# blasif/cocons

Measured on AMD Instinct MI355X. Metric: -2loglik evals/sec (dense cov_rns + Cholesky/solve/log-det, fp64) at n=10000, higher is better.
Workload: dtype f64

## Files before the change

### cocons_amd/csrc/api.hip

```cpp
#include "fit.hpp"

thread_local std::string g_err;

int fail(int code, const char *fmt, ...)
{
    char buf[512];
    va_list ap;
    va_start(ap, fmt);
    vsnprintf(buf, sizeof buf, fmt, ap);
    va_end(ap);
    g_err = buf;
    return code;
}

extern "C" const char *cocons_last_error(void) { return g_err.c_str(); }
extern "C" int cocons_abi_version(void) { return 1; }

extern "C" int cocons_device_count(void)
{
    int n = 0;
    hipError_t e = hipGetDeviceCount(&n);
    if (e != hipSuccess) { g_err = hipGetErrorString(e); return -1; }
    return n;
}
// ... 271 lines not shown
        CK(hipMemcpyAsync(f->dxb, x_betas, (size_t)n * q * sizeof(double), hipMemcpyHostToDevice, f->stream));
    }
    CK(hipStreamSynchronize(f->stream));
    CK(f->dloc.alloc((size_t)LOCP_FIELDS * f->npad));
    CK(f->dinv.alloc(2 * 8 * 256));
    int nr_max = r + (q > p ? q : p);
    f->out_cap = (size_t)(1 + nr_max * nr_max) * (size_t)(f->nt + 2);
    {
        double *hbase = nullptr;
        CK(f->dinfo_out.alloc(f->out_cap + 1));
        CK(hipHostMalloc(&hbase, (f->out_cap + 2) * sizeof(double)));
        f->dinfo = (int *)f->dinfo_out.get(); f->dout = f->dinfo_out + 1;
        f->hinfo = (int *)hbase; f->hout = hbase + 1;
        f->hinfo_init = (int *)(hbase + 1 + f->out_cap);
        f->hinfo_init[0] = 0x7f7f7f7f; f->hinfo_init[1] = 0;
    }
    for (auto &e : f->ev) CK(hipEventCreate(&e));
    f->engine_ok = want_engine;
    CK(hipEventCreateWithFlags(&f->ev_eng, hipEventDisableTiming));
    if (!defer_matrix && fit_alloc_matrix(f, nr_max) != 0) { cocons_fit_destroy(f); return nullptr; }
#undef CK
    if (engine_warm(f) != 0) { cocons_fit_destroy(f); return nullptr; }
    if (return_locked) f->op_mu.lock();
    registry_add(f);
    return f;
}

extern "C" cocons_fit *cocons_fit_create(int n, int p, int r, int q, const double *locs,
                                         const double *X, const double *z, const double *x_betas,
                                         const double *smooth_limits, int device)
// ... 215 lines not shown
    FIT_ENTER(f);
    HIPCHK(hipStreamSynchronize(f->stream));
    if (f->stream2) HIPCHK(hipStreamSynchronize(f->stream2));
    if (f->own_stream) { HIPCHK(hipStreamDestroy(f->stream)); f->own_stream = false; }
    f->stream = (hipStream_t)stream;
    return 0;
}

extern "C" int cocons_fit_sync(cocons_fit *f)
{
    FIT_ENTER(f);
    HIPCHK(hipStreamSynchronize(f->stream));
    return 0;
}

void assemble_sigma(cocons_fit *f, const double *theta, int which, int col0, int col1)
{
    ThetaVecs tv;
    make_theta_vecs(theta, f->p, tv);
    ModeSel ms = select_mode(theta, f->p, f->smooth_limits, which);
    launch_loc_params(loc_args(f->n, f->p, f->dX, f->dlocs, f->dloc, f->npad, tv, ms.smooth_kind, f->smooth_limits), f->stream);
    PairArgs pa;
    memset(&pa, 0, sizeof pa);
    pa.n = f->n; pa.m = f->n;
    pa.rows = f->dloc; pa.cols = f->dloc;
    pa.stride = f->npad; pa.stride_rows = f->npad;
    pa.out = f->dA; pa.ld = f->lda;
    pa.nrows_out = f->npad; pa.ncols_out = col1;
    pa.bj0 = col0 / 64;
    if (pa.bj0 < f->pad0 / 64) pa.bj0 = f->pad0 / 64;
    pa.pad_diag = f->nslot > 0 ? 1e300 : 1.0;
    pa.gr = ms.gr; pa.nu_fixed = ms.nu_fixed;
    launch_pair_sym(ms.mode, false, pa, f->stream);
}

int assemble_sigma_taper(cocons_fit *f, const double *theta)
{
    ThetaVecs tv;
    make_theta_vecs(theta, f->p, tv, true);
    ModeSel ms = select_mode(theta, f->p, f->smooth_limits, 0);
    launch_loc_params(loc_args(f->n, f->p, f->dX, f->dlocs, f->dloc, f->npad, tv, ms.smooth_kind, f->smooth_limits), f->stream);
    if (f->d_thi) launch_band_zero(f->dA, f->lda, f->d_thi, f->nt, f->taper_maxband, f->stream, f->skew);
    else HIPCHK(hipMemsetAsync(f->dA, 0, f->lda * (size_t)f->npad * sizeof(double), f->stream));
    TaperLaunch t;
    t.mode = ms.mode; t.nrows = f->n; t.nnz = f->taper_nnz; t.ci = f->d_tci; t.rp = f->d_trp; t.nu_fixed = ms.nu_fixed;
    t.rows = t.cols = f->dloc; t.stride_rows = t.stride = f->npad;
    t.tapv = f->d_tval; t.A = f->dA; t.lda = f->lda; t.skew = f->skew; t.npad = f->npad;
    launch_taper(t, f->stream);
    launch_pad_identity(f->dA, f->lda, f->n, f->npad, f->stream, f->skew);
    return 0;
}

int no_taper(cocons_fit *f, const char *who)
{
    if (f->taper_nnz > 0) return fail(-1, "%s: not available on a taper fit (cocons_neg2loglik_dense is)", who);
    return 0;
}

void assemble_rhs(cocons_fit *f, const double *mean, bool use_trend, const double *xb, int nxb,
                  int col0, int col1, bool zero_rest, bool slots)
{
    if (slots) { zero_rest = false; col1 = f->n; }
    RhsArgs ra;
    memset(&ra, 0, sizeof ra);
    ra.n = f->n; ra.p = f->p; ra.X = f->dX; ra.ldx = f->n;
    ra.use_trend = use_trend ? 1 : 0;
    if (use_trend) for (int i = 0; i < f->p; ++i) ra.mean[i] = canon_nan(mean[i]);
    ra.src = f->dz; ra.lds = f->n;
    ra.out = f->dA; ra.ld = f->lda;
    ra.skew = f->skew; ra.npad = f->npad;
    ra.row0 = slots ? f->n : f->npad; ra.nrows = f->r;
    ra.nrows_zero = (nxb > 0 || !zero_rest) ? 0 : f->rhs_act - f->r;
    ra.col0 = col0; ra.ncols_out = col1;
    launch_rhs_rows(ra, f->stream);
    if (nxb > 0) {
        ra.use_trend = 0;
        ra.src = xb; ra.lds = f->n;
        ra.row0 = (slots ? f->n : f->npad) + f->r; ra.nrows = nxb;
        ra.nrows_zero = zero_rest ? f->rhs_act - f->r - nxb : 0;
        launch_rhs_rows(ra, f->stream);
    }
}

FactorView main_view(cocons_fit *f)
{
    FactorView v;
    v.A = f->dA; v.lda = f->lda; v.nt = f->nt; v.mt = f->nt + f->rhs_act / TILE;
    v.hi = f->taper_hi.empty() ? nullptr : f->taper_hi.data();
    v.skew = f->skew;
    return v;
}

static RhsLayout rhs_layout(const cocons_fit *f, int nrhs)
{
    RhsLayout l;
    l.slots = f->nslot >= nrhs && f->nslot > 0;
// ... 149 lines not shown

static void count_update_flops(cocons_fit *f, int kw, int t0)
{
    double m = (double)f->n_user - ((double)t0 * TILE - (double)f->pad0);
    if (m > (double)f->n_user) m = (double)f->n_user;
    if (m < 0) m = 0;
    const double K = (double)kw * TILE - (t0 == kw ? (double)f->pad0 : 0.0);
    f->upd_flops += K * m * (m + 1.0) + 2.0 * K * (double)f->nrhs_cur * m;
}

static bool engine_wanted(cocons_fit *f, const FactorView &v)
{
    return engine_enabled() && f->engine_ok && f->stream2 != nullptr && f->engine_skip == 0 && v.nt > 4;
}

int flags_reset(cocons_fit *f, int nt)
{
    if (f->flags_cap < nt) {
        const int cap = round_up(nt + 8, 64);
        HIPCHK(f->dflags.reserve(handoff_word_count(cap), f->stream, f->stream2));
        f->flags_cap = cap;
    }
    HIPCHK(hipMemsetAsync(f->dflags, 0, handoff_word_count(f->flags_cap) * sizeof(unsigned), f->stream));
    return 0;
}

int mbox_reset(cocons_fit *f, int nt, bool engine_schedule)
{
    const MboxLayout l = mbox_layout(nt, tun().panel_fused && tun().engine_pair, tun().panel_split != 0);
    HIPCHK(f->dmbox.reserve(l.total(), f->stream, f->stream2));
    f->mbox = l;
    HIPCHK(hipMemsetAsync(f->dmbox, 0xff, (engine_schedule ? l.total() : l.tiles) * sizeof(double), f->stream));
    return 0;
}

static int engine_warm(cocons_fit *f)
{
    if (!engine_enabled() || f->nt <= 4 || !f->engine_ok) { f->engine_ok = f->engine_ok && f->stream2 != nullptr; return 0; }
    if (!f->stream2) HIPCHK(hipStreamCreateWithFlags(&f->stream2, hipStreamNonBlocking));
    if (int rc = flags_reset(f, f->nt)) return rc;
    HIPCHK(hipStreamSynchronize(f->stream));
    {
        std::vector<hipStream_t> losers;
        int ok = 0;
        for (int attempt = 0; attempt < 8; ++attempt) {
            ok = streams_run_concurrently(f->stream2, f->stream, handoff_words(f).selftest);
            if (ok != 0) break;
            losers.push_back(f->stream2);
            f->stream2 = nullptr;
// ... 87 lines not shown
                                                tun().dag_order ? tun().dag_bw : 0, tun().dag_bh);
        HIPCHK(hipStreamSynchronize(f->stream));
        if (f->stream2) HIPCHK(hipStreamSynchronize(f->stream2));
        HIPCHK(f->ddag_steps.reserve(steps.size() + 1, f->stream, f->stream2, -1, true));
        HIPCHK(hipMemcpyAsync(f->ddag_steps, steps.data(), steps.size() * sizeof(DagStepHost), hipMemcpyHostToDevice, f->stream));
        HIPCHK(f->ddag_ftab.reserve(ftab.size(), f->stream, f->stream2));
        if (!ftab.empty())
            HIPCHK(hipMemcpyAsync(f->ddag_ftab, ftab.data(), ftab.size() * sizeof(unsigned), hipMemcpyHostToDevice, f->stream));
        f->dag_xcd_g = want_tab ? xcd_g : 0;
        f->dag_have_ftab = want_tab && !ftab.empty();
        HIPCHK(hipStreamSynchronize(f->stream));
        f->dag_nsteps = (int)steps.size(); f->dag_ntasks = ntasks;
        memcpy(f->dag_key, key, sizeof key);
        HIPCHK(f->ddag.reserve(dag_words(f, v.mt).total, f->stream, f->stream2));
    }
    HIPCHK(hipMemsetAsync(f->ddag, 0, f->ddag.count() * sizeof(unsigned), f->stream));
    const size_t trace_elems = dag_trace_words(f, v.nt).count;
    if (tun().dag_trace) HIPCHK(f->ddag_trace.reserve(trace_elems, f->stream, f->stream2));
    f->dag_trace_tasks = (tun().dag_trace && f->ddag_trace) ? f->dag_ntasks : 0;
    if (f->dag_trace_tasks)
        HIPCHK(hipMemsetAsync(f->ddag_trace, 0, trace_elems * sizeof(unsigned long long), f->stream));
    return 0;
}

extern "C" long long cocons_debug_dag_trace(cocons_fit *f, int *nsteps_out, int *steps_out, unsigned long long *stamps_out,
                                            unsigned long long *engine_out)
{
    FIT_ENTER(f);
    if (!f->ddag_steps) return fail(-1, "cocons_debug_dag_trace: no DAG factorisation on this handle yet");
    if (nsteps_out) *nsteps_out = f->dag_nsteps;
    HIPCHK(hipStreamSynchronize(f->stream));
// ... 26 lines not shown
    const DagWords w = dag_words(f, v.mt);
    DagLaunch d;
    d.A = v.A; d.lda = v.lda; d.P = f->dP; d.Wt = f->dWt; d.steps = f->ddag_steps; d.nsteps = f->dag_nsteps; d.ntasks = f->dag_ntasks;
    d.queue = w.queue; d.tdone = w.tdone; d.pdone = w.pdone; d.pstride = w.pstride; d.pall = w.pall; d.dcount = w.dcount; d.xcnt = w.xcnt;
    d.partbuf = f->dpart; d.sig = hw.in; d.out = hw.out; d.xr = hw.xr; d.abort_word = hw.abort;
    d.alive = alive; d.xcc_quota = dag_xcc_quota(); d.xcd_g = f->dag_xcd_g;
    if (f->dag_have_ftab) d.ftab = f->ddag_ftab;
    return d;
}

static int engine_start(cocons_fit *f, const FactorView &v)
{
    if (f->engine_live) return 0;
    const int nt = v.nt;
    hipStream_t M = f->stream;
    if (int rc = flags_reset(f, nt)) return rc;
    f->dag_next = dag_wanted(f, v);
    if (f->dag_next) {
        if (int rc = dag_prepare(f, v)) return rc;
        if (f->dag_nsteps < 2) f->dag_next = false;
    }
    f->engine_pair_live = tun().engine_pair != 0 ? 1 : 0;
    if (f->engine_pair_live || (tun().potrf_follow && !f->follow_off))
        if (int rc = mbox_reset(f, nt > f->nt ? nt : f->nt)) return rc;
    HIPCHK(hipEventRecord(f->ev_eng, M));
    HIPCHK(hipStreamWaitEvent(f->stream2, f->ev_eng, 0));
    const HandoffWords hw = handoff_words(f);
    EngineLaunch e;
    e.A = v.A; e.lda = v.lda; e.nt = nt; e.dinv = f->dinv; e.info = f->dinfo; e.in_wait_ms = tun().engine_in_wait_ms;
    e.in = hw.in; e.out = hw.out; e.xr = hw.xr; e.abort_word = hw.abort; e.alive = hw.alive;
    if (f->dag_next) { e.wbuf = f->dWt; e.pbuf = f->dP; e.dag_until = 2 * f->dag_nsteps; }
    if (f->dag_next && f->dag_trace_tasks) e.trace = dag_trace_words(f, nt).engine;
    if (f->engine_pair_live) e.mbox = f->dmbox;
    launch_potrf_engine(e, f->stream2);
    f->engine_live = true;
    return 0;
}

int factorize(cocons_fit *f, const FactorView &v, std::vector<hipEvent_t> *ev_upd)
{
    const int nt = v.nt, mt = v.mt;
    hipStream_t M = f->stream;
    launch_front_identity(v.A, v.lda, f->pad0, mt * TILE, M);
    f->follow_used = false;
    if (!engine_wanted(f, v)) {
        f->engine_used = false;
        f->dag_used = false;
        if (int rc = flags_reset(f, nt)) return rc;
        if (tun().potrf_follow && !f->follow_off)
            if (int rc = mbox_reset(f, nt > f->nt ? nt : f->nt, false)) return rc;
        if (v.hi) {
            for (int k = 0; k < nt; ++k) {
                const int hb = v.hi[k] < nt ? v.hi[k] : nt;
                double *q = f->dinv + (size_t)(k & 1) * 2048;
                double *Ak = band_base(v.A, k, v.skew);
                const int e0 = v.skew ? k + v.skew : nt, e1 = e0 + (mt - nt);
                RowRange rows;
                rows.r0 = (k + 1) * TILE; rows.r1 = e1 * TILE - 64 * v.trim; rows.band_r1 = hb * TILE; rows.ext_r0 = e0 * TILE;
                potrf_solve(f, Ak, v.lda, k, rows, q, M);
                if (k + 1 < nt) {
                    UpdateLaunch u = v.update(hb);
                    u.panel_in_c(k * TILE); u.K = TILE; u.ti0 = k + 1; u.ti1 = mt; u.tj0 = k + 1; u.tj1 = hb < nt ? hb : nt; u.lower_only = true;
                    u.skew = v.skew;
                    launch_update(u, M);
                }
// ... 82 lines not shown
{
    HIPCHK(hipMemcpyAsync(f->dinfo, f->hinfo_init, 2 * sizeof(int), hipMemcpyHostToDevice, f->stream));
    return 0;
}

static int enqueue_eval_impl(cocons_fit *f, const double *theta, const double *mean, bool use_trend,
                             const double *xb, int nxb, std::vector<hipEvent_t> *ev_upd, bool stage_events)
{
    const int nrhs = f->r + nxb;
    f->nrhs_cur = nrhs;
    const int was_clean = f->border_clean;
    const double *was_A = f->dA;
    if (int rc = fit_alloc_matrix(f, nrhs)) return rc;
    const bool zero_rest = !(was_clean == nrhs && was_A == f->dA);
    f->border_pending = nrhs;
    if (stage_events) hipEventRecord(f->ev[0], f->stream);
    if (int rc = reset_info(f)) return rc;
    if (f->taper_nnz > 0) { if (int rc = assemble_sigma_taper(f, theta)) return rc; }
    else assemble_sigma(f, theta, 0, 0, f->npad);
    const RhsLayout lay = rhs_layout(f, nrhs);
    const bool slots = lay.slots;
    FactorView fv = rhs_view(f, lay);
    fv.dag_ok = true;
    if (engine_wanted(f, fv))
        if (int rc = engine_start(f, fv)) return rc;
    assemble_rhs(f, mean, use_trend, xb, nxb, 0, f->npad, zero_rest, slots);
    if (stage_events) hipEventRecord(f->ev[1], f->stream);
    if (int rc = factorize(f, fv, ev_upd)) return rc;
    if (stage_events) hipEventRecord(f->ev[2], f->stream);
    launch_finalize(f->dA, f->lda, f->n, slots ? f->n : f->npad, nrhs, f->dout, f->stream, f->skew, f->npad,
                    f->dag_used ? f->dP : nullptr, f->dag_used ? 2 * TILE * f->dag_nsteps : 0);
    HIPCHK(hipMemcpyAsync(f->hinfo, f->dinfo, (size_t)(2 + nrhs * nrhs) * sizeof(double),
                          hipMemcpyDeviceToHost, f->stream));
    if (stage_events) hipEventRecord(f->ev[3], f->stream);
    HIPCHK(hipGetLastError());
    return 0;
}

static int enqueue_eval(cocons_fit *f, const double *theta, const double *mean, bool use_trend,
                        const double *xb, int nxb, std::vector<hipEvent_t> *ev_upd, bool stage_events)
{
    struct timespec t0, t1;
    clock_gettime(CLOCK_MONOTONIC, &t0);
    const int rc = enqueue_eval_impl(f, theta, mean, use_trend, xb, nxb, ev_upd, stage_events);
    clock_gettime(CLOCK_MONOTONIC, &t1);
    f->enq_host_us += (t1.tv_sec - t0.tv_sec) * 1e6 + (t1.tv_nsec - t0.tv_nsec) * 1e-3;
    f->enq_calls++;
    return rc;
// ... 726 lines not shown
```

### cocons_amd/csrc/api_shard.hip

```cpp
#include <dlfcn.h>
#include <thread>
#include "fit.hpp"

struct RcclApi {
    void *h;
    ncclResult_t (*GetUniqueId)(ncclUniqueId *);
    ncclResult_t (*CommInitRank)(ncclComm_t *, int, ncclUniqueId, int);
    ncclResult_t (*CommInitAll)(ncclComm_t *, int, const int *);
    ncclResult_t (*CommDestroy)(ncclComm_t);
    ncclResult_t (*Broadcast)(const void *, void *, size_t, ncclDataType_t, int, ncclComm_t, hipStream_t);
    ncclResult_t (*AllReduce)(const void *, void *, size_t, ncclDataType_t, ncclRedOp_t, ncclComm_t, hipStream_t);
    ncclResult_t (*AllGather)(const void *, void *, size_t, ncclDataType_t, ncclComm_t, hipStream_t);
    ncclResult_t (*GroupStart)();
    ncclResult_t (*GroupEnd)();
    const char *(*GetErrorString)(ncclResult_t);
    ncclResult_t (*CommCount)(const ncclComm_t, int *);
    ncclResult_t (*CommUserRank)(const ncclComm_t, int *);
    ncclResult_t (*CommCuDevice)(const ncclComm_t, int *);
    ncclResult_t (*CommAbort)(ncclComm_t);
    ncclResult_t (*Send)(const void *, size_t, ncclDataType_t, int, ncclComm_t, hipStream_t);
    ncclResult_t (*Recv)(void *, size_t, ncclDataType_t, int, ncclComm_t, hipStream_t);
    ncclResult_t (*CommSplit)(ncclComm_t, int, int, ncclComm_t *, void *);
};

// ... 146 lines not shown
        if (!S->ev_comm_L[b]) HIPCHK(hipEventCreateWithFlags(&S->ev_comm_L[b], hipEventDisableTiming));
        if (!S->ev_main_X[b]) HIPCHK(hipEventCreateWithFlags(&S->ev_main_X[b], hipEventDisableTiming));
        if (!S->ev_comm_X[b]) HIPCHK(hipEventCreateWithFlags(&S->ev_comm_X[b], hipEventDisableTiming));
        if (!S->ev_main_U[b]) HIPCHK(hipEventCreateWithFlags(&S->ev_main_U[b], hipEventDisableTiming));
        S->unpacked[b] = false;
    }
    if (!S->ev_main_L) HIPCHK(hipEventCreateWithFlags(&S->ev_main_L, hipEventDisableTiming));
    return 0;
}

static int shard_begin(cocons_fit *f, const double *theta, const double *mean, int rank, int world)
{
    if (int rc = no_taper(f, "sharded evaluation")) return rc;
    if (f->r < 1) return fail(-1, "sharded evaluation: fit has no z");
    if (int rc = shard_prepare(f, rank, world)) return rc;
    if (int rc = reset_info(f)) return rc;
    if (engine_enabled()) {
        if (int rc = flags_reset(f, f->nt)) return rc;
        if (tun().engine_pair)
            if (int rc = mbox_reset(f, f->nt)) return rc;
    }
    ThetaVecs tv;
    make_theta_vecs(theta, f->p, tv);
    ModeSel ms = select_mode(theta, f->p, f->smooth_limits, 0);
    launch_loc_params(loc_args(f->n, f->p, f->dX, f->dlocs, f->dloc, f->npad, tv, ms.smooth_kind, f->smooth_limits),
                      f->stream);
    PairArgs pa;
    pa.n = f->n; pa.m = f->n; pa.rows = f->dloc; pa.cols = f->dloc;
    pa.stride = f->npad; pa.stride_rows = f->npad; pa.out = f->dA; pa.ld = f->lda;
    pa.nrows_out = f->npad; pa.ncols_out = f->npad;
    pa.bj0 = f->pad0 / 64; pa.H = 0; pa.blocked = 0;
    pa.gr = ms.gr; pa.nu_fixed = ms.nu_fixed;
    pa.pad_diag = f->nslot > 0 ? 1e300 : 1.0;
    pa.own_world = world; pa.own_rank = rank; pa.own_group = shard_group();
    launch_pair_sym(ms.mode, false, pa, f->stream);
    const int mt = f->nt + f->rhs_act / TILE;
    if (shard_owner(f->nt / PT, world) == rank)
        assemble_rhs(f, mean, true, nullptr, 0, 0, f->npad);
    launch_front_identity(f->dA, f->lda, f->pad0, mt * TILE, f->stream);
    HIPCHK(hipGetLastError());
    return 0;
// ... 541 lines not shown
```

### cocons_amd/csrc/assemble.hip

```cpp
#include <hip/hip_runtime.h>
#include <stdlib.h>
#include "kernels.h"
#include "matern_device.hpp"

namespace cocons {

__global__ void __launch_bounds__(256)
loc_params_kernel(LocArgs a)
{
    int w = blockIdx.x * blockDim.x + threadIdx.x;
    if (w >= a.n) return;
    const int p = a.p;
    double t_tilt = 0, t_rd = 0, t_an = 0, t_dets = 0, t_sig = 0, t_ng = 0, t_sm = 0, t_sd = 0;
    for (int i = 0; i < p; ++i) {
        double x = a.X[w + (size_t)i * a.ldx];
        t_tilt = fma(x, a.th.tilt[i], t_tilt);
        t_rd = fma(x, a.th.two_scale_je[i], t_rd);
        t_an = fma(x, a.th.aniso[i], t_an);
        t_dets = fma(x, a.th.sqrt_vector[i], t_dets);
        t_sig = fma(x, a.th.half_sd[i], t_sig);
        t_ng = fma(x, a.th.nugget[i], t_ng);
        t_sm = fma(x, a.th.smooth[i], t_sm);
        t_sd = fma(x, a.th.sd[i], t_sd);
    }
    const double pi = 3.14159265358979323846;
// ... 114 lines not shown
            cl = wave * (TS / 4) + cc;
        }
        const int r = blockIdx.x * TS + rl;
        const int c = blockIdx.y * TS + cl;
        if (c >= a.ncols_out) continue;
        double v = 0.0;
        if (r < m && c < a.n) {
            int rr = r;
            asm volatile("" : "+v"(rr));
            v = pair_value_idx<MODE>(a.rows, a.stride_rows, rr, a.cols, a.stride, c, a.gr, a.nu_fixed, true);
        }
        if (r < a.nrows_out) a.out[(size_t)r + (size_t)c * a.ld] = v;
    }
}

__global__ void __launch_bounds__(256)
rhs_rows_kernel(RhsArgs a)
{
    int c = a.col0 + blockIdx.x * blockDim.x + threadIdx.x;
    if (c >= a.ncols_out) return;
    double trend = 0.0;
    if (a.use_trend && c < a.n) {
        for (int i = 0; i < a.p; ++i) trend += a.X[c + (size_t)i * a.ldx] * a.mean[i];
    }
    for (int k = 0; k < a.nrows; ++k) {
        double v = 0.0;
        if (c < a.n) v = a.src[c + (size_t)k * a.lds] - trend;
        a.out[band_index(a.row0 + k, c, a.ld, a.skew, a.npad)] = v;
    }
    for (int k = a.nrows; k < a.nrows + a.nrows_zero; ++k)
        a.out[band_index(a.row0 + k, c, a.ld, a.skew, a.npad)] = 0.0;
}

struct TaperArgs {
    int nrows, nnz;
    const int *ci, *rp;
    const double *rows; size_t stride_rows;
    const double *cols; size_t stride;
    double nu_fixed;
    double *out;
    const double *tapv; double *A; size_t lda; int row0;
    int skew, npad;
};

template <int MODE, bool PRED>
__global__ void __launch_bounds__(256, PAIR_MIN_WAVES)
// ... 60 lines not shown

__global__ void __launch_bounds__(256)
front_identity_kernel(double *A, size_t lda, int pad0, int rows)
{
    const int r = blockIdx.x * blockDim.x + threadIdx.x, c = blockIdx.y;
    if (r < c || r >= rows || c >= pad0) return;
    A[(size_t)r + (size_t)c * lda] = (r == c) ? 1.0 : 0.0;
}

void launch_front_identity(double *A, size_t lda, int pad0, int rows, hipStream_t s)
{
    if (pad0 > 0 && rows > 0)
        hipLaunchKernelGGL(front_identity_kernel, dim3((rows + 255) / 256, pad0), dim3(256), 0, s, A, lda, pad0, rows);
}

void launch_pad_identity(double *A, size_t lda, int n, int npad, hipStream_t s, int skew)
{
    if (npad > n)
        hipLaunchKernelGGL(pad_identity_kernel, dim3((npad - n + 255) / 256), dim3(256), 0, s, A, lda, n, npad, skew);
}

struct RowsArgs {
    int n, nidx;
    const int *idx;
    const double *loc; size_t stride;
    double gr, nu_fixed;
    int cor;
    double *out;
};

// ... 112 lines not shown
```

### cocons_amd/csrc/fit.hpp

```cpp
#pragma once
#include <hip/hip_runtime.h>
#include <limits.h>
#include <math.h>
#include <stdarg.h>
#include <stdint.h>
#include <stdio.h>
#include <stdlib.h>
#include <string.h>
#include <unistd.h>
#include <time.h>
#include <rccl/rccl.h>

#include <algorithm>
#include <limits>
#include <memory>
#include <mutex>
#include <string>
#include <vector>

#include "kernels.h"
#include "../../include/cocons_hip_diag.h"
#include "matern_device.hpp"

using namespace cocons;
// ... 189 lines not shown
    int npad = 0, nt = 0;
    int rhs_cap = 0;
    int rhs_act = 0;
    size_t lda = 0;
    hipStream_t stream = nullptr;
    bool own_stream = false;
    DevBuf<double> dX, dlocs, dz, dxb;
    DevBuf<double> dloc;
    DevBuf<double> dA;
    DevBuf<double> dinv;
    DevBuf<double> dinfo_out;
    int *dinfo = nullptr;
    double *dout = nullptr;
    double *hout = nullptr;
    int *hinfo = nullptr, *hinfo_init = nullptr;
    double smooth_limits[2] = {0, 0};
    size_t out_cap = 0;
    DevBuf<double> dlocp, dXp, dlocsp, dstoch, dquad, dred;
    int rank = 0, world = 1, nrhs_cur = 0;
    int nslot = 0;
    int n_user = 0, pad0 = 0;
    DevBuf<double> xbuf[2];
    hipEvent_t ev[8] = {};
    hipStream_t stream2 = nullptr;
    hipEvent_t ev_eng = nullptr;
    DevBuf<unsigned> dflags;
    int flags_cap = 0;
    bool engine_ok = false;
    bool engine_live = false;
    bool engine_used = false;
    int border_clean = -1;
    int border_pending = -1;
    bool engine_active_last = false;
    int engine_skip = 0;
    int engine_fails = 0;
    int engine_retries = 0;
    int engine_last_abort = 0;
    long long engine_ops = 0;
    DevBuf<double> dP;
    DevBuf<double> dWt;
    DevBuf<double> dpart;
    DevBuf<unsigned> ddag;
    DevBuf<DagStepHost> ddag_steps; int dag_nsteps = 0; unsigned dag_ntasks = 0;
    int dag_key[12] = {};
// ... 179 lines not shown
    int dag_trace = 0;
    int gate_sabotage = 0;
    int host_delay_us = 0, host_delay_tile = -1, engine_in_wait_ms = 0;
    bool init = false;
};

Tunables &tun();
bool engine_enabled();
int fit_alloc_matrix(cocons_fit *f, int rhs_rows);
cocons_fit *fit_create_impl(int n, int p, int r, int q, const double *locs, const double *X, const double *z, const double *x_betas,
                            const double *smooth_limits, int device, bool allow_sort, bool defer_matrix = false,
                            bool want_engine = true, bool return_locked = false);
cocons_fit *taper_create_ordered(int n, int p, int r, const double *locs, const double *X, const double *z,
                                 const double *smooth_limits, int device, int nnz, const int *colindices, const int *rowpointers,
                                 const double *taper_entries, const std::vector<int> &perm, bool check_fit);
void assemble_sigma(cocons_fit *f, const double *theta, int which, int col0, int col1);
int assemble_sigma_taper(cocons_fit *f, const double *theta);
int no_taper(cocons_fit *f, const char *who);
void assemble_rhs(cocons_fit *f, const double *mean, bool use_trend, const double *xb, int nxb, int col0, int col1,
                  bool zero_rest = true, bool slots = false);
FactorView main_view(cocons_fit *f);
int flags_reset(cocons_fit *f, int nt);
int mbox_reset(cocons_fit *f, int nt, bool engine_schedule = true);
int factorize(cocons_fit *f, const FactorView &v, std::vector<hipEvent_t> *ev_upd);
int reset_info(cocons_fit *f);
int info_status(cocons_fit *f);
bool engine_retry(cocons_fit *f, int st);
void dense_collect(cocons_fit *f, double *sum_logliks, double *parts);
int profile_tail(cocons_fit *f, int nxb, double n_eff, bool reml, double *sum_logliks, double *parts);
int sharded_eval(cocons_fit *f, const double *theta, const double *mean, double *sum_logliks, double *parts);
void shard_events_destroy(ShardState *S);
void rccl_comm_destroy(ncclComm_t c);

size_t grad_lda(const cocons_fit *f, int nb);
int grad_prepare(cocons_fit *f, const char *who, int nb, int pcols = 0);
int grad_enqueue(cocons_fit *f, const double *theta, const double *mean, bool full, double *hgrad);
int taper_grad_prepare(cocons_fit *f, const char *who);
int taper_grad_enqueue(cocons_fit *f, const double *theta, const double *mean, double *hgrad);
// ... 35 lines not shown
```

### cocons_amd/csrc/kernels.h

```cpp
#pragma once
#include <hip/hip_runtime.h>
#include <stddef.h>
#include <atomic>
#include <vector>
#include "../../include/cocons_hip.h"

namespace cocons {

enum SmoothKind : int {
    SMOOTH_ZERO = 0,
    SMOOTH_LOGISTIC_SQRT = 1,
    SMOOTH_EXP = 2
};

struct ThetaVecs {
    double tilt[COCONS_P_MAX];
    double two_scale_je[COCONS_P_MAX];
    double aniso[COCONS_P_MAX];
    double sqrt_vector[COCONS_P_MAX];
    double half_sd[COCONS_P_MAX];
    double nugget[COCONS_P_MAX];
    double smooth[COCONS_P_MAX];
    double sd[COCONS_P_MAX];
};

struct LocArgs {
    int n, p;
    const double *X; int ldx;
    const double *locs; int ldl;
    double *out; size_t stride;
    int smooth_kind;
    double smooth_min, smooth_max;
    ThetaVecs th;
};

struct PairArgs {
    int n;
    int m;
    const double *rows;
    const double *cols;
    size_t stride;
    size_t stride_rows;
    double *out; size_t ld;
    int nrows_out, ncols_out;
    int bj0;
    int H;
    int blocked;
    double gr;
// ... 7 lines not shown
    const double *X; int ldx;
    double mean[COCONS_P_MAX];
    int use_trend;
    const double *src; int lds;
    double *out; size_t ld;
    int row0, nrows;
    int nrows_zero;
    int col0, ncols_out;
    int skew, npad;
};

void launch_loc_params(const LocArgs &a, hipStream_t s);
void launch_pair_sym(int mode, bool mirror, const PairArgs &a, hipStream_t s);
void launch_pair_rect(int mode, const PairArgs &a, hipStream_t s);
void launch_rhs_rows(const RhsArgs &a, hipStream_t s);
struct TaperLaunch {
    int mode = 0; bool pred = false;
    int nrows = 0, nnz = 0; const int *ci = nullptr, *rp = nullptr;
    const double *rows = nullptr; size_t stride_rows = 0;
    const double *cols = nullptr; size_t stride = 0;
    double nu_fixed = 0.0; double *out = nullptr;
    const double *tapv = nullptr; double *A = nullptr; size_t lda = 0; int row0 = 0;
    int skew = 0, npad = 0;
};
void launch_taper(const TaperLaunch &t, hipStream_t s);
void launch_band_zero(double *A, size_t lda, const int *d_hi, int nt, int max_band, hipStream_t s, int skew = 0);
void launch_front_identity(double *A, size_t lda, int pad0, int rows, hipStream_t s);
void launch_pad_identity(double *A, size_t lda, int n, int npad, hipStream_t s, int skew = 0);
void launch_cov_rows(int mode, int n, int nidx, const int *idx, const double *loc, size_t stride, double gr,
                     double nu_fixed, int cor, double *out, hipStream_t s);
// ... 99 lines not shown
    double *A = nullptr; size_t lda = 0; double *P = nullptr; const double *Wt = nullptr;
    const DagStepHost *steps = nullptr; int nsteps = 0; unsigned ntasks = 0;
    unsigned *queue = nullptr, *tdone = nullptr, *pdone = nullptr; int pstride = 0; unsigned *pall = nullptr;
    double *partbuf = nullptr; unsigned *dcount = nullptr;
    unsigned *sig = nullptr, *out = nullptr, *xr = nullptr, *abort_word = nullptr;
    unsigned long long *trace = nullptr; unsigned *hw = nullptr;
    const unsigned *alive = nullptr; int xcc_quota = 0;
    const unsigned *ftab = nullptr; int xcd_g = 0;
    unsigned *xcnt = nullptr;
};
void launch_dag(const DagLaunch &d, hipStream_t s);

void launch_finalize(const double *A, size_t lda, int n, int row0, int nr, double *out, hipStream_t s,
                     int skew = 0, int npad = 0,
                     const double *A2 = nullptr,
                     int a2_cols = 0);
void launch_finalize_cols(const double *A, size_t lda, int c0, int c1, int n, int row0, int nr,
                          double *out, hipStream_t s);
size_t row_reduce_scratch_doubles(int n, int m);
void launch_row_reduce(const double *A, size_t lda, int n, int rowy, int row0, int m,
                       double *stoch, double *quad, double *scratch, hipStream_t s, int skew = 0, int npad = 0,
                       const double *A2 = nullptr, int a2_cols = 0);

void launch_trmm_lower(const double *A, size_t lda, int n, const double *E, int lde, int nsim,
                       const double *trend, double *Y, int ldy, hipStream_t s);
void launch_band_trmm(const double *A, size_t lda, int skew, int npad, const int *d_hi, int nt, int n, const double *E,
                      int lde, int nsim, const double *trend, double *Y, int ldy, hipStream_t s);
void launch_krige_pack(const double *A, size_t lda, int nt, int rowy, int c_lo, int c_hi, double *Lp, double *Qp, double *w,
                       hipStream_t s);
void launch_krige_solve(const double *Lp, const double *Qp, const double *w, int nt, double *C, size_t ldc, int rows,
                        int c_lo, int c_hi, double *stoch, double *quad, hipStream_t s);
// ... 103 lines not shown
```

### cocons_amd/csrc/solve.hip

```cpp
#include <hip/hip_runtime.h>
#include <algorithm>
#include <atomic>
#include "kernels.h"
#include "tile_ops.hpp"

namespace cocons {

__device__ __forceinline__ double block_sum(double v, double *red)
{
#pragma unroll
    for (int o = 32; o > 0; o >>= 1) v += __shfl_down(v, o, 64);
    int lane = threadIdx.x & 63, wave = threadIdx.x >> 6;
    if (lane == 0) red[wave] = v;
    __syncthreads();
    double t = 0.0;
    if (threadIdx.x == 0)
        for (int w = 0; w < (int)(blockDim.x >> 6); ++w) t += red[w];
    __syncthreads();
    return t;
}

__global__ void __launch_bounds__(1024)
finalize_kernel(const double *A, size_t lda, int c0, int c1, int n, int row0, int nr, double *out, int skew, int npad,
                const double *A2, int a2_cols)
{
    __shared__ double red[16];
    const int b = blockIdx.x;
    const int hi = c1 < n ? c1 : n;
    double s = 0.0;
    constexpr int U = 4;
    const int step = (int)blockDim.x;
    if (b == nr * nr) {
        for (int c = c0 + (int)threadIdx.x; c < hi; c += U * step) {
            double v[U];
#pragma unroll
            for (int q = 0; q < U; ++q) v[q] = (c + q * step < hi) ? A[band_index(c + q * step, c + q * step, lda, skew, npad)] : 1.0;
#pragma unroll
            for (int q = 0; q < U; ++q) s += log(v[q]);
        }
    } else {
        const int ra = row0 + b / nr, rb = row0 + b % nr;
        for (int c = c0 + (int)threadIdx.x; c < hi; c += U * step) {
            double va[U], vb[U];
#pragma unroll
            for (int q = 0; q < U; ++q) {
// ... 41 lines not shown
    const int i = blockIdx.x * blockDim.x + threadIdx.x;
    if (i >= m) return;
    double s = 0.0, q = 0.0;
    for (int c = 0; c < nchunks; ++c) {
        s += scratch[((size_t)c * 2 + 0) * m + i];
        q += scratch[((size_t)c * 2 + 1) * m + i];
    }
    stoch[i] = s;
    quad[i] = q;
}

void launch_finalize_cols(const double *A, size_t lda, int c0, int c1, int n, int row0, int nr,
                          double *out, hipStream_t s)
{
    hipLaunchKernelGGL(finalize_kernel, dim3(nr * nr + 1), dim3(1024), 0, s, A, lda, c0, c1, n, row0, nr, out, 0, 0,
                       (const double *)nullptr, 0);
}

void launch_finalize(const double *A, size_t lda, int n, int row0, int nr, double *out, hipStream_t s, int skew, int npad,
                     const double *A2, int a2_cols)
{
    hipLaunchKernelGGL(finalize_kernel, dim3(nr * nr + 1), dim3(1024), 0, s, A, lda, 0, n, n, row0, nr, out, skew, npad,
                       skew ? (const double *)nullptr : A2, a2_cols);
}

size_t row_reduce_scratch_doubles(int n, int m)
{
    return (size_t)2 * (size_t)m * (size_t)((n + 255) / 256);
}

void launch_row_reduce(const double *A, size_t lda, int n, int rowy, int row0, int m,
                       double *stoch, double *quad, double *scratch, hipStream_t s, int skew, int npad,
                       const double *A2, int a2_cols)
{
    if (m <= 0) return;
    const int cchunk = 2 * TILE, nchunks = (n + cchunk - 1) / cchunk;
    hipLaunchKernelGGL(row_reduce_kernel, dim3((m + 255) / 256, nchunks), dim3(256), 0, s,
                       A, lda, n, rowy, row0, m, scratch, cchunk, skew, npad, skew ? (const double *)nullptr : A2, a2_cols);
// ... 595 lines not shown
```

Baseline: 125.1.

## Fold eval-time resets, border fills and result copy into fewer kernel launches

The per-evaluation info reset moves into the loc_params kernel. The flags, dag and mbox memsets merge into a single multi-segment reset kernel, and the RHS row writes are combined with the front-identity fill in one border kernel. The finalize kernel now writes results and the info words straight into mapped host memory, which removes the device-to-host memcpy, and its unroll factor rises from 4 to 16. The aim is to cut launch and memset overhead per evaluation, at the cost of zero-copy host writes and more state coupling through front_live.

```diff
diff --git a/cocons_amd/csrc/api.hip b/cocons_amd/csrc/api.hip
--- a/cocons_amd/csrc/api.hip
+++ b/cocons_amd/csrc/api.hip
@@ -309,6 +309,9 @@
         f->hinfo = (int *)hbase; f->hout = hbase + 1;
         f->hinfo_init = (int *)(hbase + 1 + f->out_cap);
         f->hinfo_init[0] = 0x7f7f7f7f; f->hinfo_init[1] = 0;
+        void *dbase = nullptr;
+        CK(hipHostGetDevicePointer(&dbase, hbase, 0));
+        f->hinfo_dev = (int *)dbase; f->hout_dev = (double *)dbase + 1;
     }
     for (auto &e : f->ev) CK(hipEventCreate(&e));
     f->engine_ok = want_engine;
@@ -554,12 +557,14 @@
     return 0;
 }
 
-void assemble_sigma(cocons_fit *f, const double *theta, int which, int col0, int col1)
+void assemble_sigma(cocons_fit *f, const double *theta, int which, int col0, int col1, bool open_eval)
 {
     ThetaVecs tv;
     make_theta_vecs(theta, f->p, tv);
     ModeSel ms = select_mode(theta, f->p, f->smooth_limits, which);
-    launch_loc_params(loc_args(f->n, f->p, f->dX, f->dlocs, f->dloc, f->npad, tv, ms.smooth_kind, f->smooth_limits), f->stream);
+    LocArgs la = loc_args(f->n, f->p, f->dX, f->dlocs, f->dloc, f->npad, tv, ms.smooth_kind, f->smooth_limits);
+    if (open_eval) la.info_reset = f->dinfo;
+    launch_loc_params(la, f->stream);
     PairArgs pa;
     memset(&pa, 0, sizeof pa);
     pa.n = f->n; pa.m = f->n;
@@ -574,12 +579,14 @@
     launch_pair_sym(ms.mode, false, pa, f->stream);
 }
 
-int assemble_sigma_taper(cocons_fit *f, const double *theta)
+int assemble_sigma_taper(cocons_fit *f, const double *theta, bool open_eval)
 {
     ThetaVecs tv;
     make_theta_vecs(theta, f->p, tv, true);
     ModeSel ms = select_mode(theta, f->p, f->smooth_limits, 0);
-    launch_loc_params(loc_args(f->n, f->p, f->dX, f->dlocs, f->dloc, f->npad, tv, ms.smooth_kind, f->smooth_limits), f->stream);
+    LocArgs la = loc_args(f->n, f->p, f->dX, f->dlocs, f->dloc, f->npad, tv, ms.smooth_kind, f->smooth_limits);
+    if (open_eval) la.info_reset = f->dinfo;
+    launch_loc_params(la, f->stream);
     if (f->d_thi) launch_band_zero(f->dA, f->lda, f->d_thi, f->nt, f->taper_maxband, f->stream, f->skew);
     else HIPCHK(hipMemsetAsync(f->dA, 0, f->lda * (size_t)f->npad * sizeof(double), f->stream));
     TaperLaunch t;
@@ -598,10 +605,13 @@
 }
 
 void assemble_rhs(cocons_fit *f, const double *mean, bool use_trend, const double *xb, int nxb,
-                  int col0, int col1, bool zero_rest, bool slots)
+                  int col0, int col1, bool zero_rest, bool slots, const FactorView *front)
 {
     if (slots) { zero_rest = false; col1 = f->n; }
-    RhsArgs ra;
+    BorderLaunch bl;
+    memset(&bl.rhs[1], 0, sizeof bl.rhs[1]);
+    if (front) { bl.A = front->A; bl.lda = front->lda; bl.pad0 = f->pad0; bl.rows = front->mt * TILE; }
+    RhsArgs &ra = bl.rhs[0];
     memset(&ra, 0, sizeof ra);
     ra.n = f->n; ra.p = f->p; ra.X = f->dX; ra.ldx = f->n;
     ra.use_trend = use_trend ? 1 : 0;
@@ -612,14 +622,15 @@
     ra.row0 = slots ? f->n : f->npad; ra.nrows = f->r;
     ra.nrows_zero = (nxb > 0 || !zero_rest) ? 0 : f->rhs_act - f->r;
     ra.col0 = col0; ra.ncols_out = col1;
-    launch_rhs_rows(ra, f->stream);
     if (nxb > 0) {
-        ra.use_trend = 0;
-        ra.src = xb; ra.lds = f->n;
-        ra.row0 = (slots ? f->n : f->npad) + f->r; ra.nrows = nxb;
-        ra.nrows_zero = zero_rest ? f->rhs_act - f->r - nxb : 0;
-        launch_rhs_rows(ra, f->stream);
-    }
+        RhsArgs &rb = bl.rhs[1];
+        rb = ra;
+        rb.use_trend = 0;
+        rb.src = xb; rb.lds = f->n;
+        rb.row0 = (slots ? f->n : f->npad) + f->r; rb.nrows = nxb;
+        rb.nrows_zero = zero_rest ? f->rhs_act - f->r - nxb : 0;
+    }
+    launch_border(bl, f->stream);
 }
 
 FactorView main_view(cocons_fit *f)
@@ -799,25 +810,29 @@
     return engine_enabled() && f->engine_ok && f->stream2 != nullptr && f->engine_skip == 0 && v.nt > 4;
 }
 
-int flags_reset(cocons_fit *f, int nt)
+int words_reset(cocons_fit *f, int nt, bool dag, int mbox)
 {
     if (f->flags_cap < nt) {
         const int cap = round_up(nt + 8, 64);
         HIPCHK(f->dflags.reserve(handoff_word_count(cap), f->stream, f->stream2));
         f->flags_cap = cap;
     }
-    HIPCHK(hipMemsetAsync(f->dflags, 0, handoff_word_count(f->flags_cap) * sizeof(unsigned), f->stream));
-    return 0;
-}
-
-int mbox_reset(cocons_fit *f, int nt, bool engine_schedule)
-{
-    const MboxLayout l = mbox_layout(nt, tun().panel_fused && tun().engine_pair, tun().panel_split != 0);
-    HIPCHK(f->dmbox.reserve(l.total(), f->stream, f->stream2));
-    f->mbox = l;
-    HIPCHK(hipMemsetAsync(f->dmbox, 0xff, (engine_schedule ? l.total() : l.tiles) * sizeof(double), f->stream));
-    return 0;
-}
+    ResetLaunch r;
+    r.seg[0].p = f->dflags.get(); r.seg[0].bytes = handoff_word_count(f->flags_cap) * sizeof(unsigned);
+    if (dag) { r.seg[1].p = f->ddag.get(); r.seg[1].bytes = f->ddag.count() * sizeof(unsigned); }
+    if (mbox != MBOX_NONE) {
+        const int tiles = nt > f->nt ? nt : f->nt;
+        const MboxLayout l = mbox_layout(tiles, tun().panel_fused && tun().engine_pair, tun().panel_split != 0);
+        HIPCHK(f->dmbox.reserve(l.total(), f->stream, f->stream2));
+        f->mbox = l;
+        r.seg[2].p = f->dmbox.get(); r.seg[2].bytes = (mbox == MBOX_ALL ? l.total() : l.tiles) * sizeof(double);
+        r.seg[2].pattern = 0xffffffffu;
+    }
+    launch_reset_words(r, f->stream);
+    return 0;
+}
+
+int flags_reset(cocons_fit *f, int nt) { return words_reset(f, nt, false, MBOX_NONE); }
 
 static int engine_warm(cocons_fit *f)
 {
@@ -935,7 +950,6 @@
         memcpy(f->dag_key, key, sizeof key);
         HIPCHK(f->ddag.reserve(dag_words(f, v.mt).total, f->stream, f->stream2));
     }
-    HIPCHK(hipMemsetAsync(f->ddag, 0, f->ddag.count() * sizeof(unsigned), f->stream));
     const size_t trace_elems = dag_trace_words(f, v.nt).count;
     if (tun().dag_trace) HIPCHK(f->ddag_trace.reserve(trace_elems, f->stream, f->stream2));
     f->dag_trace_tasks = (tun().dag_trace && f->ddag_trace) ? f->dag_ntasks : 0;
@@ -992,15 +1006,14 @@
     if (f->engine_live) return 0;
     const int nt = v.nt;
     hipStream_t M = f->stream;
-    if (int rc = flags_reset(f, nt)) return rc;
     f->dag_next = dag_wanted(f, v);
     if (f->dag_next) {
         if (int rc = dag_prepare(f, v)) return rc;
         if (f->dag_nsteps < 2) f->dag_next = false;
     }
     f->engine_pair_live = tun().engine_pair != 0 ? 1 : 0;
-    if (f->engine_pair_live || (tun().potrf_follow && !f->follow_off))
-        if (int rc = mbox_reset(f, nt > f->nt ? nt : f->nt)) return rc;
+    const bool want_mbox = f->engine_pair_live || (tun().potrf_follow && !f->follow_off);
+    if (int rc = words_reset(f, nt, f->dag_next, want_mbox ? MBOX_ALL : MBOX_NONE)) return rc;
     HIPCHK(hipEventRecord(f->ev_eng, M));
     HIPCHK(hipStreamWaitEvent(f->stream2, f->ev_eng, 0));
     const HandoffWords hw = handoff_words(f);
@@ -1019,14 +1032,13 @@
 {
     const int nt = v.nt, mt = v.mt;
     hipStream_t M = f->stream;
-    launch_front_identity(v.A, v.lda, f->pad0, mt * TILE, M);
+    if (f->front_live) f->front_live = false;
+    else launch_front_identity(v.A, v.lda, f->pad0, mt * TILE, M);
     f->follow_used = false;
     if (!engine_wanted(f, v)) {
         f->engine_used = false;
         f->dag_used = false;
-        if (int rc = flags_reset(f, nt)) return rc;
-        if (tun().potrf_follow && !f->follow_off)
-            if (int rc = mbox_reset(f, nt > f->nt ? nt : f->nt, false)) return rc;
+        if (int rc = words_reset(f, nt, false, (tun().potrf_follow && !f->follow_off) ? MBOX_TILES : MBOX_NONE)) return rc;
         if (v.hi) {
             for (int k = 0; k < nt; ++k) {
                 const int hb = v.hi[k] < nt ? v.hi[k] : nt;
@@ -1139,24 +1151,23 @@
     if (int rc = fit_alloc_matrix(f, nrhs)) return rc;
     const bool zero_rest = !(was_clean == nrhs && was_A == f->dA);
     f->border_pending = nrhs;
+    f->front_live = false;
     if (stage_events) hipEventRecord(f->ev[0], f->stream);
-    if (int rc = reset_info(f)) return rc;
-    if (f->taper_nnz > 0) { if (int rc = assemble_sigma_taper(f, theta)) return rc; }
-    else assemble_sigma(f, theta, 0, 0, f->npad);
+    if (f->taper_nnz > 0) { if (int rc = assemble_sigma_taper(f, theta, true)) return rc; }
+    else assemble_sigma(f, theta, 0, 0, f->npad, true);
     const RhsLayout lay = rhs_layout(f, nrhs);
     const bool slots = lay.slots;
     FactorView fv = rhs_view(f, lay);
     fv.dag_ok = true;
     if (engine_wanted(f, fv))
         if (int rc = engine_start(f, fv)) return rc;
-    assemble_rhs(f, mean, use_trend, xb, nxb, 0, f->npad, zero_rest, slots);
+    assemble_rhs(f, mean, use_trend, xb, nxb, 0, f->npad, zero_rest, slots, &fv);
+    f->front_live = true;
     if (stage_events) hipEventRecord(f->ev[1], f->stream);
     if (int rc = factorize(f, fv, ev_upd)) return rc;
     if (stage_events) hipEventRecord(f->ev[2], f->stream);
-    launch_finalize(f->dA, f->lda, f->n, slots ? f->n : f->npad, nrhs, f->dout, f->stream, f->skew, f->npad,
-                    f->dag_used ? f->dP : nullptr, f->dag_used ? 2 * TILE * f->dag_nsteps : 0);
-    HIPCHK(hipMemcpyAsync(f->hinfo, f->dinfo, (size_t)(2 + nrhs * nrhs) * sizeof(double),
-                          hipMemcpyDeviceToHost, f->stream));
+    launch_finalize(f->dA, f->lda, f->n, slots ? f->n : f->npad, nrhs, f->hout_dev, f->stream, f->skew, f->npad,
+                    f->dag_used ? f->dP : nullptr, f->dag_used ? 2 * TILE * f->dag_nsteps : 0, f->dinfo, f->hinfo_dev);
     if (stage_events) hipEventRecord(f->ev[3], f->stream);
     HIPCHK(hipGetLastError());
     return 0;
diff --git a/cocons_amd/csrc/api_shard.hip b/cocons_amd/csrc/api_shard.hip
--- a/cocons_amd/csrc/api_shard.hip
+++ b/cocons_amd/csrc/api_shard.hip
@@ -184,17 +184,14 @@
     if (int rc = no_taper(f, "sharded evaluation")) return rc;
     if (f->r < 1) return fail(-1, "sharded evaluation: fit has no z");
     if (int rc = shard_prepare(f, rank, world)) return rc;
-    if (int rc = reset_info(f)) return rc;
-    if (engine_enabled()) {
-        if (int rc = flags_reset(f, f->nt)) return rc;
-        if (tun().engine_pair)
-            if (int rc = mbox_reset(f, f->nt)) return rc;
-    }
+    if (engine_enabled())
+        if (int rc = words_reset(f, f->nt, false, tun().engine_pair ? MBOX_ALL : MBOX_NONE)) return rc;
     ThetaVecs tv;
     make_theta_vecs(theta, f->p, tv);
     ModeSel ms = select_mode(theta, f->p, f->smooth_limits, 0);
-    launch_loc_params(loc_args(f->n, f->p, f->dX, f->dlocs, f->dloc, f->npad, tv, ms.smooth_kind, f->smooth_limits),
-                      f->stream);
+    LocArgs la = loc_args(f->n, f->p, f->dX, f->dlocs, f->dloc, f->npad, tv, ms.smooth_kind, f->smooth_limits);
+    la.info_reset = f->dinfo;
+    launch_loc_params(la, f->stream);
     PairArgs pa;
     pa.n = f->n; pa.m = f->n; pa.rows = f->dloc; pa.cols = f->dloc;
     pa.stride = f->npad; pa.stride_rows = f->npad; pa.out = f->dA; pa.ld = f->lda;
diff --git a/cocons_amd/csrc/assemble.hip b/cocons_amd/csrc/assemble.hip
--- a/cocons_amd/csrc/assemble.hip
+++ b/cocons_amd/csrc/assemble.hip
@@ -9,6 +9,7 @@
 loc_params_kernel(LocArgs a)
 {
     int w = blockIdx.x * blockDim.x + threadIdx.x;
+    if (w == 0 && a.info_reset) { a.info_reset[0] = 0x7f7f7f7f; a.info_reset[1] = 0; }
     if (w >= a.n) return;
     const int p = a.p;
     double t_tilt = 0, t_rd = 0, t_an = 0, t_dets = 0, t_sig = 0, t_ng = 0, t_sm = 0, t_sd = 0;
@@ -153,10 +154,9 @@
     }
 }
 
-__global__ void __launch_bounds__(256)
-rhs_rows_kernel(RhsArgs a)
-{
-    int c = a.col0 + blockIdx.x * blockDim.x + threadIdx.x;
+__device__ __forceinline__ void rhs_rows_body(const RhsArgs &a, int block, int pad0, int rows)
+{
+    int c = a.col0 + block * (int)blockDim.x + threadIdx.x;
     if (c >= a.ncols_out) return;
     double trend = 0.0;
     if (a.use_trend && c < a.n) {
@@ -165,10 +165,17 @@
     for (int k = 0; k < a.nrows; ++k) {
         double v = 0.0;
         if (c < a.n) v = a.src[c + (size_t)k * a.lds] - trend;
+        if (c < pad0 && a.row0 + k < rows) v = 0.0;
         a.out[band_index(a.row0 + k, c, a.ld, a.skew, a.npad)] = v;
     }
     for (int k = a.nrows; k < a.nrows + a.nrows_zero; ++k)
         a.out[band_index(a.row0 + k, c, a.ld, a.skew, a.npad)] = 0.0;
+}
+
+__global__ void __launch_bounds__(256)
+rhs_rows_kernel(RhsArgs a)
+{
+    rhs_rows_body(a, blockIdx.x, 0, 0);
 }
 
 struct TaperArgs {
@@ -259,6 +266,80 @@
         hipLaunchKernelGGL(front_identity_kernel, dim3((rows + 255) / 256, pad0), dim3(256), 0, s, A, lda, pad0, rows);
 }
 
+struct BorderArgs {
+    RhsArgs rhs[2];
+    int nb0, nb1;
+    double *A; size_t lda; int pad0, rows, rblocks;
+};
+
+__global__ void __launch_bounds__(256)
+border_kernel(BorderArgs a)
+{
+    int b = blockIdx.x;
+    if (b < a.nb0) { rhs_rows_body(a.rhs[0], b, a.pad0, a.rows); return; }
+    b -= a.nb0;
+    if (b < a.nb1) { rhs_rows_body(a.rhs[1], b, a.pad0, a.rows); return; }
+    b -= a.nb1;
+    const int c = b / a.rblocks, r = (b % a.rblocks) * (int)blockDim.x + threadIdx.x;
+    if (r < c || r >= a.rows || c >= a.pad0) return;
+    a.A[(size_t)r + (size_t)c * a.lda] = (r == c) ? 1.0 : 0.0;
+}
+
+static int rhs_blocks(const RhsArgs &a)
+{
+    const int nc = a.ncols_out - a.col0;
+    return (nc <= 0 || a.nrows + a.nrows_zero <= 0) ? 0 : (nc + 255) / 256;
+}
+
+void launch_border(const BorderLaunch &l, hipStream_t s)
+{
+    BorderArgs a;
+    a.rhs[0] = l.rhs[0]; a.rhs[1] = l.rhs[1];
+    a.nb0 = rhs_blocks(l.rhs[0]); a.nb1 = rhs_blocks(l.rhs[1]);
+    const bool front = l.pad0 > 0 && l.rows > 0;
+    a.A = l.A; a.lda = l.lda; a.pad0 = front ? l.pad0 : 0; a.rows = front ? l.rows : 0;
+    a.rblocks = front ? (l.rows + 255) / 256 : 1;
+    const int nb = a.nb0 + a.nb1 + (front ? a.rblocks * a.pad0 : 0);
+    if (nb > 0) hipLaunchKernelGGL(border_kernel, dim3(nb), dim3(256), 0, s, a);
+}
+
+struct ResetArgs {
+    unsigned *p[3]; size_t bytes[3]; unsigned pattern[3];
+};
+
+__global__ void __launch_bounds__(256)
+reset_words_kernel(ResetArgs a)
+{
+#pragma unroll
+    for (int q = 0; q < 4; ++q) {
+        size_t i = ((size_t)blockIdx.x * 4 + q) * 256 + threadIdx.x;
+        bool done = false;
+#pragma unroll
+        for (int g = 0; g < 3; ++g) {
+            const size_t units = (a.bytes[g] + 15) / 16;
+            if (!done && i < units) {
+                const unsigned v = a.pattern[g];
+                if (16 * (i + 1) <= a.bytes[g]) *(uint4 *)(a.p[g] + 4 * i) = make_uint4(v, v, v, v);
+                else for (size_t w = 4 * i; w < a.bytes[g] / 4; ++w) a.p[g][w] = v;
+                done = true;
+            }
+            if (!done) i -= units;
+        }
+    }
+}
+
+void launch_reset_words(const ResetLaunch &r, hipStream_t s)
+{
+    ResetArgs a;
+    size_t units = 0;
+    for (int g = 0; g < 3; ++g) {
+        const bool on = r.seg[g].p != nullptr && r.seg[g].bytes > 0;
+        a.p[g] = on ? (unsigned *)r.seg[g].p : nullptr; a.bytes[g] = on ? r.seg[g].bytes : 0; a.pattern[g] = r.seg[g].pattern;
+        units += (a.bytes[g] + 15) / 16;
+    }
+    if (units > 0) hipLaunchKernelGGL(reset_words_kernel, dim3((unsigned)((units + 1023) / 1024)), dim3(256), 0, s, a);
+}
+
 void launch_pad_identity(double *A, size_t lda, int n, int npad, hipStream_t s, int skew)
 {
     if (npad > n)
diff --git a/cocons_amd/csrc/fit.hpp b/cocons_amd/csrc/fit.hpp
--- a/cocons_amd/csrc/fit.hpp
+++ b/cocons_amd/csrc/fit.hpp
@@ -227,6 +227,8 @@
     double *dout = nullptr;
     double *hout = nullptr;
     int *hinfo = nullptr, *hinfo_init = nullptr;
+    int *hinfo_dev = nullptr;
+    double *hout_dev = nullptr;
     double smooth_limits[2] = {0, 0};
     size_t out_cap = 0;
     DevBuf<double> dlocp, dXp, dlocsp, dstoch, dquad, dred;
@@ -241,6 +243,7 @@
     int flags_cap = 0;
     bool engine_ok = false;
     bool engine_live = false;
+    bool front_live = false;
     bool engine_used = false;
     int border_clean = -1;
     int border_pending = -1;
@@ -450,14 +453,15 @@
 cocons_fit *taper_create_ordered(int n, int p, int r, const double *locs, const double *X, const double *z,
                                  const double *smooth_limits, int device, int nnz, const int *colindices, const int *rowpointers,
                                  const double *taper_entries, const std::vector<int> &perm, bool check_fit);
-void assemble_sigma(cocons_fit *f, const double *theta, int which, int col0, int col1);
-int assemble_sigma_taper(cocons_fit *f, const double *theta);
+void assemble_sigma(cocons_fit *f, const double *theta, int which, int col0, int col1, bool open_eval = false);
+int assemble_sigma_taper(cocons_fit *f, const double *theta, bool open_eval = false);
 int no_taper(cocons_fit *f, const char *who);
 void assemble_rhs(cocons_fit *f, const double *mean, bool use_trend, const double *xb, int nxb, int col0, int col1,
-                  bool zero_rest = true, bool slots = false);
+                  bool zero_rest = true, bool slots = false, const FactorView *front = nullptr);
 FactorView main_view(cocons_fit *f);
+enum { MBOX_NONE = 0, MBOX_TILES = 1, MBOX_ALL = 2 };
+int words_reset(cocons_fit *f, int nt, bool dag, int mbox);
 int flags_reset(cocons_fit *f, int nt);
-int mbox_reset(cocons_fit *f, int nt, bool engine_schedule = true);
 int factorize(cocons_fit *f, const FactorView &v, std::vector<hipEvent_t> *ev_upd);
 int reset_info(cocons_fit *f);
 int info_status(cocons_fit *f);
diff --git a/cocons_amd/csrc/kernels.h b/cocons_amd/csrc/kernels.h
--- a/cocons_amd/csrc/kernels.h
+++ b/cocons_amd/csrc/kernels.h
@@ -32,6 +32,7 @@
     int smooth_kind;
     double smooth_min, smooth_max;
     ThetaVecs th;
+    int *info_reset = nullptr;
 };
 
 struct PairArgs {
@@ -69,6 +70,18 @@
 void launch_pair_sym(int mode, bool mirror, const PairArgs &a, hipStream_t s);
 void launch_pair_rect(int mode, const PairArgs &a, hipStream_t s);
 void launch_rhs_rows(const RhsArgs &a, hipStream_t s);
+struct BorderLaunch {
+    RhsArgs rhs[2];
+    double *A = nullptr; size_t lda = 0; int pad0 = 0, rows = 0;
+};
+void launch_border(const BorderLaunch &b, hipStream_t s);
+struct WordFill {
+    void *p = nullptr; size_t bytes = 0; unsigned pattern = 0;
+};
+struct ResetLaunch {
+    WordFill seg[3];
+};
+void launch_reset_words(const ResetLaunch &r, hipStream_t s);
 struct TaperLaunch {
     int mode = 0; bool pred = false;
     int nrows = 0, nnz = 0; const int *ci = nullptr, *rp = nullptr;
@@ -198,7 +211,9 @@
 void launch_finalize(const double *A, size_t lda, int n, int row0, int nr, double *out, hipStream_t s,
                      int skew = 0, int npad = 0,
                      const double *A2 = nullptr,
-                     int a2_cols = 0);
+                     int a2_cols = 0,
+                     const int *info_src = nullptr,
+                     int *info_dst = nullptr);
 void launch_finalize_cols(const double *A, size_t lda, int c0, int c1, int n, int row0, int nr,
                           double *out, hipStream_t s);
 size_t row_reduce_scratch_doubles(int n, int m);
diff --git a/cocons_amd/csrc/solve.hip b/cocons_amd/csrc/solve.hip
--- a/cocons_amd/csrc/solve.hip
+++ b/cocons_amd/csrc/solve.hip
@@ -22,13 +22,14 @@
 
 __global__ void __launch_bounds__(1024)
 finalize_kernel(const double *A, size_t lda, int c0, int c1, int n, int row0, int nr, double *out, int skew, int npad,
-                const double *A2, int a2_cols)
+                const double *A2, int a2_cols, const int *info_src, int *info_dst)
 {
     __shared__ double red[16];
     const int b = blockIdx.x;
     const int hi = c1 < n ? c1 : n;
     double s = 0.0;
-    constexpr int U = 4;
+    if (info_dst && b == 0 && threadIdx.x == 64) { info_dst[0] = info_src[0]; info_dst[1] = info_src[1]; }
+    constexpr int U = 16;
     const int step = (int)blockDim.x;
     if (b == nr * nr) {
         for (int c = c0 + (int)threadIdx.x; c < hi; c += U * step) {
@@ -100,14 +101,14 @@
                           double *out, hipStream_t s)
 {
     hipLaunchKernelGGL(finalize_kernel, dim3(nr * nr + 1), dim3(1024), 0, s, A, lda, c0, c1, n, row0, nr, out, 0, 0,
-                       (const double *)nullptr, 0);
+                       (const double *)nullptr, 0, (const int *)nullptr, (int *)nullptr);
 }
 
 void launch_finalize(const double *A, size_t lda, int n, int row0, int nr, double *out, hipStream_t s, int skew, int npad,
-                     const double *A2, int a2_cols)
+                     const double *A2, int a2_cols, const int *info_src, int *info_dst)
 {
     hipLaunchKernelGGL(finalize_kernel, dim3(nr * nr + 1), dim3(1024), 0, s, A, lda, 0, n, n, row0, nr, out, skew, npad,
-                       skew ? (const double *)nullptr : A2, a2_cols);
+                       skew ? (const double *)nullptr : A2, a2_cols, info_src, info_dst);
 }
 
 size_t row_reduce_scratch_doubles(int n, int m)
```

After: 124.1. About the same (-0.8%).
